# vqdang/hover_net

Measured on AMD Instinct MI355X. Metric: tiles/sec (270x270, batch 32) end-to-end incl. watershed, higher is better.
Workload: dtype fp32

## Files before the change

### hover_net_amd/csrc/hvn_api.hip

```cpp
#include <hip/hip_runtime.h>
#include <stdarg.h>
#include <stdio.h>
#include <string.h>

#include <vector>

#include "hvn_kernels.h"

static thread_local char g_err[512] = "";

int hvn_fail(int code, const char *fmt, ...)
{
    va_list ap;
    va_start(ap, fmt);
    vsnprintf(g_err, sizeof(g_err), fmt, ap);
    va_end(ap);
    return code;
}

int hvn_launch_status(int rc, const char *what)
{
    return rc ? hvn_fail(rc, "%s: %s", what, rc == HVN_E_LAUNCH ? "launch failed" : "the launcher refused these arguments") : HVN_OK;
}

// ... 102 lines not shown

static int nbr_common(const char *what, const hvn_op *op, int batch)
{
    const int N = op->x.h;
    if (!op->w || !op->x2.base) return hvn_fail(HVN_E_ARG, "%s: null pointer", what);
    if (batch != 1) return hvn_fail(HVN_E_ARG, "%s: batch %d, not 1", what, batch);
    if (((uintptr_t)op->w & 7) || ((uintptr_t)op->x2.base & 7)) return hvn_fail(HVN_E_ARG, "%s: misaligned table or workspace (8)", what);
    if (N < 1) return hvn_fail(HVN_E_ARG, "%s: N = %d, fewer than one point", what, N);
    if (op->kh < 1 || op->kw < 1) return hvn_fail(HVN_E_ARG, "%s: a grid of %d x %d cells", what, op->kh, op->kw);
    if (N > HVN_NBR_MAX_N) return hvn_fail(HVN_E_SIZE, "%s: N = %d above 2^26", what, N);
    const long cells = (long)op->kh * op->kw;
    if (op->kh > HVN_NBR_MAX_AXIS || op->kw > HVN_NBR_MAX_AXIS || cells > HVN_NBR_MAX_CELLS)
        return hvn_fail(HVN_E_SIZE, "%s: a grid of %d x %d cells, more than 4096 per axis or 2^22 in all", what, op->kh, op->kw);
    if ((long)op->x2.sn < HVN_NBR_WORKSPACE_BYTES(N, cells))
        return hvn_fail(HVN_E_SIZE, "%s: workspace of %ld bytes, %ld needed", what, (long)op->x2.sn, HVN_NBR_WORKSPACE_BYTES(N, cells));
    return 0;
}

int hvn_internal_run_one(const hvn_op *op, int batch, hipStream_t s)
{
    switch (op->kind) {
    case HVN_OP_CONV0: {
        Conv0Args a;
        set_view(op->x, a.img, a.isn, a.isy, a.isx);
        a.isc = op->x.sc ? op->x.sc : 1;
        a.is_f32 = op->x_dtype;
        a.H = op->x.h; a.W = op->x.w;
        a.w = op->w; a.bias = op->bias;
        set_view(op->y, a.y, a.ysn, a.ysy, a.ysx);
        a.N = batch; a.Ho = op->y.h; a.Wo = op->y.w; a.pad = op->pad_t; a.relu = op->relu; a.out_bf16 = op->act_dtype == 1;
        if (op->kh != 7 || op->kw != 7 || op->x.c != 3 || op->y.c != 64 || !op->w || !op->bias || !op->x.base || !op->y.base)
            return hvn_fail(HVN_E_ARG, "conv0: expects 7x7x3->64 with bias, a non-null image and output");
        if (!aligned16(a.y) || !strides_ok(op->y, 3)) return hvn_fail(HVN_E_ARG, "conv0: output view not 16-byte aligned");
        return hvn_launch_status(hvn_launch_conv0(a, s), "conv0");
    }
    case HVN_OP_CONV: {
        ConvArgs a;
        memset(&a, 0, sizeof(a));
        set_view(op->x, a.x, a.xsn, a.xsy, a.xsx);
        a.H = op->x.h; a.W = op->x.w; a.Cin = op->x.c;
        a.w = op->w; a.bias = op->bias;
        a.pre_s = op->pre_scale; a.pre_b = op->pre_shift;
        a.post_s = op->post_scale; a.post_b = op->post_shift;
        set_view(op->res, a.res, a.rsn, a.rsy, a.rsx);
        set_view(op->y, a.y, a.ysn, a.ysy, a.ysx);
        a.N = batch; a.Ho = op->y.h; a.Wo = op->y.w; a.Cout = op->cout;
        a.KH = op->kh; a.KW = op->kw; a.stride = op->stride; a.pad_t = op->pad_t; a.pad_l = op->pad_l;
        a.relu = op->relu;
        a.groups = op->groups > 1 ? op->groups : 1;
        set_view(op->x2, a.x2, a.x2sn, a.x2sy, a.x2sx);
        a.Cin2 = a.x2 ? op->x2.c : 0;
        a.stride2 = op->_rsv > 0 ? op->_rsv : 1;
        if (a.x2 && (op->kh != 1 || op->kw != 1 || a.stride != 1 || a.Cin2 % 32 || !aligned16(a.x2) || !strides_ok(op->x2, 3) ||
                     a.pre_s || (long)(a.Ho - 1) * a.stride2 >= op->x2.h || (long)(a.Wo - 1) * a.stride2 >= op->x2.w))
            return hvn_fail(HVN_E_ARG, "conv: second input needs a 1x1 stride-1 op without prologue and a view that covers the output grid");
        a.M = (long)batch * a.Ho * a.Wo;
        if (!a.x || !a.w || !a.y) return hvn_fail(HVN_E_ARG, "conv: null pointer");
        if (a.Cin % 32) return hvn_fail(HVN_E_ARG, "conv: input channels must be a multiple of 32 (got %d)", a.Cin);
        if (!aligned16(a.x) || !aligned16(a.w) || !strides_ok(op->x, 3))
            return hvn_fail(HVN_E_ARG, "conv: input view / weights not 16-byte aligned");
        if ((a.pre_s && !aligned16(a.pre_s)) || (a.pre_b && !aligned16(a.pre_b)) || (!a.pre_s != !a.pre_b))
            return hvn_fail(HVN_E_ARG, "conv: prologue vectors must be 16-byte aligned and come in pairs");
        if (!a.post_s != !a.post_b) return hvn_fail(HVN_E_ARG, "conv: epilogue affine must come in pairs");
        if (op->y.c != op->cout) return hvn_fail(HVN_E_ARG, "conv: output view channels != cout");
        a.nbatch = op->nbatch > 1 ? op->nbatch : 1;
        a.xb = op->batch_stride[0]; a.wb = op->batch_stride[1]; a.yb = op->batch_stride[2];
        if (a.nbatch > 1 && ((a.xb | a.wb | a.yb) & 3)) return hvn_fail(HVN_E_ARG, "conv: batch strides must keep 16-byte alignment");
        const bool bf16 = op->act_dtype == 1;
        if (bf16 && (!strides_ok(op->x, 7) || (a.x2 && !strides_ok(op->x2, 7)) || a.nbatch > 1))
            return hvn_fail(HVN_E_ARG, "conv(bf16): input strides must be multiples of 8 elements; no batched launch");
        if (g_prof) prof_mark(s);
        const bool x3 = op->act_dtype == 2 || op->act_dtype == 3;
        if (x3 && (a.groups > 1 || (a.nbatch > 1 && (a.wb & 7)))) return hvn_fail(HVN_E_ARG, "conv(bf16x3): no grouped convs; batch stride of the planes must keep 16-byte alignment");
        int rc;
        if (bf16 && (op->tile_n == 896 || op->tile_n == 640))
            rc = hvn_launch_conv_bf16g(a, op->tile_n == 896 ? 256 : 128, s);
        else if (bf16)
            rc = hvn_launch_conv_bf16(a, op->tile_n, s);
        else if (x3 && (op->tile_n == 896 || op->tile_n == 640))
            rc = hvn_launch_conv_x3g(a, op->tile_n == 896 ? 256 : 128, op->act_dtype == 3 ? 6 : 9, s);
        else
            rc = x3 ? hvn_launch_conv_x3(a, op->tile_n, op->act_dtype == 3 ? 6 : 9, s) : hvn_launch_conv(a, op->tile_n, s);
        if (g_prof) prof_mark(s);
        if (rc) return hvn_fail(rc, "conv: launch failed (tile_n=%d)", op->tile_n);
        return HVN_OK;
    }
    case HVN_OP_CHAIN: {
        ChainArgs a;
        memset(&a, 0, sizeof(a));
        set_view(op->x, a.x, a.xsn, a.xsy, a.xsx);
        a.K1 = op->x.c;
        set_view(op->x2, a.x2, a.x2sn, a.x2sy, a.x2sx);
        a.K1b = a.x2 ? op->x2.c : 0;
        a.stride2 = op->_rsv > 0 ? op->_rsv : 1;
        a.w1 = op->w;
        set_view(op->res, a.res, a.rsn, a.rsy, a.rsx);
        set_view(op->y, a.y, a.ysn, a.ysy, a.ysx);
        a.C = op->cout;
        a.post_s = op->post_scale; a.post_b = op->post_shift;
        a.pre_s = op->pre_scale; a.pre_b = op->pre_shift;
        a.w2 = op->w2; a.bias2 = op->bias2; a.relu2 = 1;
        set_view(op->y2, a.y2, a.y2sn, a.y2sy, a.y2sx);
        a.N2 = op->cout2;
        a.N = batch; a.Ho = op->y.h; a.Wo = op->y.w;
        a.M = (long)batch * a.Ho * a.Wo;
        a.bm = op->tile_n == 64 ? 64 : 128;
        const bool cx3 = op->act_dtype == 2 || op->act_dtype == 3;
        const bool cbf = op->act_dtype == 1;
        if (op->act_dtype != 0 && !cx3 && !cbf) return hvn_fail(HVN_E_ARG, "chain: act_dtype 0 (fp32), 1 (bf16) or 2 | 3 (fp32 with bf16x3 products)");
        const char *form = cbf ? " (bf16)" : "";
        const bool channels_ok = cbf ? hvn_chain_bf16_supported(a.K1, a.K1b, a.C, a.N2) != 0
                                     : hvn_chain_supported(a.C, a.N2) && !(a.K1 % 32 || a.K1b % 32 || a.K1 + a.K1b < 64);
        const long stride_mask = cbf ? 7 : 3;
        if (!a.x || !a.w1 || !a.y || !a.w2 || !a.y2) return hvn_fail(HVN_E_ARG, "chain: null pointer");
        if (op->kh != 1 || op->kw != 1 || op->stride != 1 || op->pad_t || op->pad_l || op->relu || op->bias)
            return hvn_fail(HVN_E_ARG, "chain: the first conv is a plain 1x1 (no bias / relu of its own)");
        if (!channels_ok || op->y.c != a.C || op->y2.c != a.N2)
            return hvn_fail(HVN_E_ARG, "chain%s: needs %s, cout2 in {64, 128} (cout2 = %d)", form,
                            cbf ? "input channels in slabs of 64 (64 or 128 in all), cout % 256 == 0" : "input channels in slabs of 32 (>= 64), cout % 64 == 0", a.N2);
        if (op->x.h != a.Ho || op->x.w != a.Wo || op->y2.h != a.Ho || op->y2.w != a.Wo ||
            (a.x2 && ((long)(a.Ho - 1) * a.stride2 >= op->x2.h || (long)(a.Wo - 1) * a.stride2 >= op->x2.w)))
            return hvn_fail(HVN_E_ARG, "chain: views do not cover the output grid");
        if (a.res && (a.rsn != a.ysn || a.rsy != a.ysy || a.rsx != a.ysx || op->res.c != a.C))
            return hvn_fail(HVN_E_ARG, "chain: the residual view must have the output's strides");
        if (!aligned16(a.x) || !aligned16(a.w1) || !aligned16(a.w2) || !aligned16(a.y) || !aligned16(a.y2) || (a.res && !aligned16(a.res)) ||
            (a.x2 && !aligned16(a.x2)) || !strides_ok(op->x, stride_mask) || !strides_ok(op->y, stride_mask) || !strides_ok(op->y2, stride_mask) ||
            !strides_ok(op->x2, stride_mask))
            return hvn_fail(HVN_E_ARG, "chain%s: views / weights not 16-byte aligned", form);
        if ((!a.pre_s != !a.pre_b) || (!a.post_s != !a.post_b) || (a.pre_s && (!aligned16(a.pre_s) || !aligned16(a.pre_b))) ||
            (a.post_s && (!aligned16(a.post_s) || !aligned16(a.post_b))) || (a.bias2 && !aligned16(a.bias2)))
            return hvn_fail(HVN_E_ARG, "chain: per-channel vectors must be 16-byte aligned and come in pairs");
        if (g_prof) prof_mark(s);
        int rc;
        if (cbf)
            rc = hvn_launch_conv_chain_bf16(a, s);
        else if (cx3 && op->tile_n == 1152)
            rc = hvn_launch_conv_chain_x3r(a, op->act_dtype == 3 ? 6 : 9, s);
        else
            rc = cx3 ? hvn_launch_conv_chain_x3(a, op->act_dtype == 3 ? 6 : 9, s) : hvn_launch_conv_chain(a, s);
        if (g_prof) prof_mark(s);
        if (rc) return hvn_fail(rc, "chain%s: launch failed (cout2=%d)", form, a.N2);
        return HVN_OK;
    }
    case HVN_OP_WINO_IN:
    case HVN_OP_WINO_OUT: {
        WinoArgs a;
        const bool in = op->kind == HVN_OP_WINO_IN;
        set_view(op->x, a.x, a.xsn, a.xsy, a.xsx);
        set_view(op->y, a.y, a.ysn, a.ysy, a.ysx);
        a.mat = op->w; a.bias = op->bias;
        a.N = batch; a.H = in ? op->x.h : op->y.h; a.W = in ? op->x.w : op->y.w; a.C = in ? op->x.c : op->y.c;
        a.ty = op->kh; a.tx = op->kw; a.pad = op->pad_t; a.relu = op->relu;
        a.accum = (!in && op->res.base != nullptr) ? 1 : 0;
        a.lo = nullptr; a.lsn = a.lsy = a.lsx = 0;
        if (in && op->res.base) {
            set_view(op->res, a.lo, a.lsn, a.lsy, a.lsx);
            if (op->res.h * 2 != op->x.h || op->res.w * 2 != op->x.w || op->res.c != op->x.c || !aligned16(a.lo) || !strides_ok(op->res, 3))
                return hvn_fail(HVN_E_ARG, "wino_in: the half-resolution input must be x.h/2 x x.w/2 x x.c and 16-byte aligned");
        }
        if (a.accum && op->res.base != op->y.base) return hvn_fail(HVN_E_ARG, "wino_out: res must alias y (accumulate in place)");
        const int n2 = in ? op->y.h : op->x.h;
        if (op->stride > 1 && op->_rsv > 1) {
            a.m = op->stride; a.r = op->_rsv;
        } else {
            a.m = n2 == 36 ? 2 : n2 == 64 ? 4 : n2 == 100 ? 6 : 0; a.r = 5;
        }
// ... 346 lines not shown
```

### hover_net_amd/csrc/hvn_conv.hip

```cpp
#include <hip/hip_runtime.h>
#include <stdint.h>
#include <stdio.h>
#include <stdlib.h>

#include <vector>

#include <type_traits>

#include "hvn_conv_common.h"

#define BK 32
#define LDS_LD 32
#ifndef HVN_TRACE_FINE
#define HVN_TRACE_FINE 0
#endif
#define HVN_TRACE_WORDS (HVN_TRACE_FINE ? 8 : 4)

template <int BM, int BN, int WAVES_M, int WAVES_N, bool PADDED, bool GROUPED = false, bool HAS_PRE = true, bool HAS_X2 = false>
__global__ __launch_bounds__(256, (BN <= 64 && BM <= 128) ? 3 : 2) void hvn_conv_igemm_f32(ConvArgs p)
{
    unsigned long long t_start = 0, t_kend = 0;
    if (p.dbg) t_start = __builtin_readcyclecounter();
    if (p.nbatch > 1) {
        p.x += (long)blockIdx.y * p.xb;
// ... 359 lines not shown
            ++e_oy;
        }
        while (e_oy >= (unsigned)p.Ho) {
            e_oy -= (unsigned)p.Ho;
            ++e_n;
        }
        const int rr = erow0 + it * RPP;
        f32x4 v = *(const f32x4 *)(ep + rr * EP_LD + ecol);
        v.x = fmaxf(v.x + bias.x, relu_lo);
        v.y = fmaxf(v.y + bias.y, relu_lo);
        v.z = fmaxf(v.z + bias.z, relu_lo);
        v.w = fmaxf(v.w + bias.w, relu_lo);
        v += rall[it];
        v.x = fmaxf(fmaf(v.x, qs.x, qb.x), post_lo);
        v.y = fmaxf(fmaf(v.y, qs.y, qb.y), post_lo);
        v.z = fmaxf(fmaf(v.z, qs.z, qb.z), post_lo);
        v.w = fmaxf(fmaf(v.w, qs.w, qb.w), post_lo);
        vout[it] = v;
    }
#pragma unroll
    for (int it = 0; it < NIT; ++it) asm volatile("" : "+v"(vout[it]), "+v"(yoffs[it]));
    __builtin_amdgcn_sched_barrier(0);
#if HVN_TRACE_FINE
    if (p.dbg) t_f[2] = __builtin_readcyclecounter();
#endif
#pragma unroll
    for (int it = 0; it < NIT; ++it)
        if (oks[it]) *(f32x4 *)(p.y + yoffs[it]) = vout[it];
#if HVN_TRACE_FINE
    if (p.dbg) t_f[3] = __builtin_readcyclecounter();
#endif
    if (p.dbg && tid == 0) {
        asm volatile("s_waitcnt vmcnt(0)" ::: "memory");
        unsigned long long *d = p.dbg + (unsigned long long)HVN_TRACE_WORDS * (blockIdx.x + (unsigned long long)gridDim.x * blockIdx.y);
#if HVN_TRACE_FINE
        d[4] = t_f[0];
        d[5] = t_f[1];
        d[6] = t_f[2];
        d[7] = t_f[3];
#endif
        d[0] = t_start;
        d[1] = t_kend;
        d[2] = __builtin_readcyclecounter();
        d[3] = (unsigned long long)__builtin_amdgcn_s_getreg(4 | (0 << 6) | ((32 - 1) << 11)) |
               ((unsigned long long)__builtin_amdgcn_s_getreg(6 | (0 << 6) | ((8 - 1) << 11)) << 32);
    }
}

template <int BM, int BN, int WAVES_M, int WAVES_N, bool PADDED, bool GROUPED = false, bool HAS_PRE = true, bool HAS_X2 = false>
static int launch_conv(const ConvArgs &a, hipStream_t stream)
{
    ConvArgs p = a;
    static unsigned long long *dbg_buf = nullptr;
    static int dbg_on = -1;
    if (dbg_on < 0) {
        dbg_on = hvn_env_str("HVN_CONV_TRACE") ? 1 : 0;
        if (dbg_on) hipMalloc(&dbg_buf, HVN_TRACE_WORDS * 8 * (size_t)(1 << 20));
    }
    p.dbg = dbg_on ? dbg_buf : nullptr;
    p.m_tiles = (p.M + BM - 1) / BM;
    p.n_tiles = (p.Cout + BN - 1) / BN;
    constexpr size_t stage_fl = (size_t)2 * (BM + BN) * LDS_LD, ep_fl = (size_t)BM * (BN + 4);
    const size_t lds = (stage_fl > ep_fl ? stage_fl : ep_fl) * sizeof(float);
    static std::atomic<unsigned long long> attr_done{0};
    auto kern = hvn_conv_igemm_f32<BM, BN, WAVES_M, WAVES_N, PADDED, GROUPED, HAS_PRE, HAS_X2>;
    if (hvn_max_lds_once((const void *)kern, (int)lds, attr_done)) return HVN_E_LAUNCH;
    const long groups = (p.m_tiles + 7) / 8;
    const long grid = groups * 8 * p.n_tiles;
    if (grid <= 0 || grid > 0x7fffffffL) return HVN_E_ARG;
    hipLaunchKernelGGL(kern, dim3((unsigned)grid, p.nbatch > 1 ? p.nbatch : 1), dim3(256), lds, stream, p);
    if (dbg_on && grid * (p.nbatch > 1 ? p.nbatch : 1) <= (1 << 20)) {
        hipStreamSynchronize(stream);
        const size_t n = (size_t)grid * (p.nbatch > 1 ? p.nbatch : 1);
        std::vector<unsigned long long> h(HVN_TRACE_WORDS * n);
        hipMemcpy(h.data(), dbg_buf, 8 * HVN_TRACE_WORDS * n, hipMemcpyDeviceToHost);
        if (FILE *f = fopen(hvn_env_str("HVN_CONV_TRACE"), "wb")) {
            fwrite(h.data(), 8, h.size(), f);
            fclose(f);
        }
    }
    return hipGetLastError() == hipSuccess ? HVN_OK : HVN_E_LAUNCH;
}

int hvn_launch_dense_grouped(const ConvArgs &a, hipStream_t stream);

int hvn_launch_conv(const ConvArgs &a, int tile_n, hipStream_t stream)
{
    if (a.Cin % BK != 0 || a.Cin <= 0 || a.Cout % 4 != 0) return HVN_E_ARG;
    const int bm = tile_n == 320 ? 256 : 128;
    if (!hvn_conv_reach_ok(a, bm, 4, 256, true, false)) return HVN_E_ARG;
    if ((long)(a.Cout + 128) * a.KH * a.KW * a.Cin * 4 >= (1L << 32)) return HVN_E_ARG;
    const bool padded = hvn_conv_padded(a);
    if (padded && a.pre_s) return HVN_E_ARG;
    if (a.x2) {
        if (padded || a.Cin2 % BK) return HVN_E_ARG;
        if (tile_n == 128) return launch_conv<128, 128, 2, 2, false, false, false, true>(a, stream);
        if (tile_n == 64) return launch_conv<128, 64, 4, 1, false, false, false, true>(a, stream);
        return HVN_E_ARG;
    }
    switch (tile_n) {
    case 128:
        if (!a.pre_s)
            return padded ? launch_conv<128, 128, 2, 2, true, false, false>(a, stream) : launch_conv<128, 128, 2, 2, false, false, false>(a, stream);
        return padded ? launch_conv<128, 128, 2, 2, true>(a, stream) : launch_conv<128, 128, 2, 2, false>(a, stream);
    case 64:
        if (!a.pre_s)
            return padded ? launch_conv<128, 64, 4, 1, true, false, false>(a, stream) : launch_conv<128, 64, 4, 1, false, false, false>(a, stream);
        return padded ? launch_conv<128, 64, 4, 1, true>(a, stream) : launch_conv<128, 64, 4, 1, false>(a, stream);
    case 320:
        if (!a.pre_s)
            return padded ? launch_conv<256, 64, 4, 1, true, false, false>(a, stream) : launch_conv<256, 64, 4, 1, false, false, false>(a, stream);
        return padded ? launch_conv<256, 64, 4, 1, true>(a, stream) : launch_conv<256, 64, 4, 1, false>(a, stream);
    case 32:
        if (a.groups == 4 && a.Cin == 128 && a.Cout == 32 && a.stride == 1 && !padded && !a.pre_s && !a.res && !a.post_s && a.nbatch <= 1 &&
            a.KH == a.KW && (a.KH == 5 || a.KH == 3))
            return hvn_launch_dense_grouped(a, stream);
        if (a.groups == 4 && a.Cin == 128 && a.Cout == 32)
            return padded ? launch_conv<128, 32, 4, 1, true, true>(a, stream) : launch_conv<128, 32, 4, 1, false, true>(a, stream);
        if (a.groups != 1 && !(a.groups == 4 && a.Cin == 128 && a.Cout == 32)) return HVN_E_ARG;
        return padded ? launch_conv<128, 32, 4, 1, true>(a, stream) : launch_conv<128, 32, 4, 1, false>(a, stream);
    default: return HVN_E_ARG;
    }
}

#define DG_TH 8
#define DG_TW 16
#define DG_PP 68
template <int KS>
__global__ __launch_bounds__(256, 2) void hvn_dense_grouped_f32(const ConvArgs p, int tiles_x, int tiles_y)
{
    constexpr int PH = DG_TH + KS - 1, PW = DG_TW + KS - 1;
    extern __shared__ __attribute__((aligned(16))) float dg_patch[];
    const int tid = threadIdx.x, lane = tid & 63, wave = tid >> 6;
    const int l15 = lane & 15, q = lane >> 4;
    int bid = blockIdx.x;
    const int gp = bid & 1;
    bid >>= 1;
    const int tx = bid % tiles_x;
    bid /= tiles_x;
    const int ty = bid % tiles_y;
    const int n = bid / tiles_y;
    const int oy0 = ty * DG_TH, ox0 = tx * DG_TW;
    const float *xin = p.x + (long)n * p.xsn + gp * 64;
    for (int i = tid; i < PH * PW * 16; i += 256) {
        const int c4 = i & 15, pix = i >> 4;
        const int py = pix / PW, px = pix - py * PW;
        const int iy = oy0 + py, ix = ox0 + px;
        f32x4 v = {0.f, 0.f, 0.f, 0.f};
        if (iy < p.H && ix < p.W) v = *(const f32x4 *)(xin + (long)iy * p.xsy + (long)ix * p.xsx + c4 * 4);
        *(f32x4 *)(dg_patch + pix * DG_PP + c4 * 4) = v;
    }
    const int gl = wave & 1, half = wave >> 1;
    const int g = 2 * gp + gl;
    const bool bvalid = l15 < 8;
    const float *wrow = p.w + ((long)(8 * g + (bvalid ? l15 : 0)) * 4 + g) * (KS * KS) * 32 + 8 * q;
    constexpr int TAPS = KS * KS;
    f32x4 wb[4][2];
#pragma unroll
    for (int t = 0; t < 4; ++t) wb[t][0] = wb[t][1] = (f32x4){0.f, 0.f, 0.f, 0.f};
    if (bvalid) {
#pragma unroll
        for (int t = 0; t < 3 && t < TAPS; ++t) {
            wb[t][0] = *(const f32x4 *)(wrow + t * 32);
            wb[t][1] = *(const f32x4 *)(wrow + t * 32 + 4);
        }
    }
    f32x4 acc[4];
#pragma unroll
    for (int m = 0; m < 4; ++m) acc[m] = (f32x4){0.f, 0.f, 0.f, 0.f};
    __syncthreads();
    const float *abase = dg_patch + ((4 * half) * PW + l15) * DG_PP + 32 * gl + 8 * q;
#pragma unroll
    for (int tap = 0; tap < TAPS; ++tap) {
        const int r = tap / KS, s2 = tap % KS;
        if (bvalid && tap + 3 < TAPS) {
            wb[(tap + 3) & 3][0] = *(const f32x4 *)(wrow + (tap + 3) * 32);
            wb[(tap + 3) & 3][1] = *(const f32x4 *)(wrow + (tap + 3) * 32 + 4);
        }
        const float *a = abase + (r * PW + s2) * DG_PP;
        f32x4 a0[4], a1[4];
#pragma unroll
        for (int m = 0; m < 4; ++m) {
            a0[m] = *(const f32x4 *)(a + m * PW * DG_PP);
            a1[m] = *(const f32x4 *)(a + m * PW * DG_PP + 4);
        }
        const f32x4 b0 = wb[tap & 3][0], b1 = wb[tap & 3][1];
#pragma unroll
        for (int e = 0; e < 4; ++e)
#pragma unroll
            for (int m = 0; m < 4; ++m) acc[m] = __builtin_amdgcn_mfma_f32_16x16x4f32(a0[m][e], b0[e], acc[m], 0, 0, 0);
#pragma unroll
        for (int e = 0; e < 4; ++e)
#pragma unroll
            for (int m = 0; m < 4; ++m) acc[m] = __builtin_amdgcn_mfma_f32_16x16x4f32(a1[m][e], b1[e], acc[m], 0, 0, 0);
    }
    if (bvalid) {
        const int co = 8 * g + l15;
        const float bias = p.bias ? p.bias[co] : 0.f;
        const float lo = p.relu ? 0.f : -__builtin_inff();
#pragma unroll
        for (int m = 0; m < 4; ++m) {
            const int oy = oy0 + 4 * half + m;
#pragma unroll
// ... 163 lines not shown
    const float lo = p.relu ? 0.f : -__builtin_inff();
    const float *acol = dg_patch + (2 * l15) * DG_PP + 32 * gl + 8 * q;
    __syncthreads();
    for (int ty = ty0; ty < ty1; ++ty) {
        const int oy0 = ty * DG2_TH;
        f32x4 pf[NPF];
        const bool more = ty + 1 < ty1;
        const int ny0 = oy0 + DG2_TH + PH - 4;
        if (more) {
#pragma unroll
            for (int j = 0; j < NPF; ++j) {
                const int i = tid + 256 * j;
                const int c4 = i & 15, pix = i >> 4;
                const int py = pix / PW, px = pix - py * PW;
                const int iy = ny0 + py, ix = ox0 + px;
                pf[j] = (f32x4){0.f, 0.f, 0.f, 0.f};
                if (i < NEW && iy < p.H && ix < p.W) pf[j] = *(const f32x4 *)(xin + (long)iy * p.xsy + (long)ix * p.xsx + c4 * 4);
            }
        }
        f32x4 wb[4][2];
#pragma unroll
        for (int t = 0; t < 3; ++t) load_w(t, wb[t][0], wb[t][1]);
        f32x4 acc[2] = {{0.f, 0.f, 0.f, 0.f}, {0.f, 0.f, 0.f, 0.f}};
        const int r0 = oy0 + 2 * half;
#pragma unroll
        for (int t2 = 0; t2 < TAPS2; ++t2) {
            const int tr = t2 / (KS + 1), tc = t2 % (KS + 1);
            if (t2 + 3 < TAPS2) load_w(t2 + 3, wb[(t2 + 3) & 3][0], wb[(t2 + 3) & 3][1]);
            f32x4 a0[2], a1[2];
#pragma unroll
            for (int m = 0; m < 2; ++m) {
                const float *a = acol + (((r0 + m + tr) & 7) * PW + tc) * DG_PP;
                a0[m] = *(const f32x4 *)(a);
                a1[m] = *(const f32x4 *)(a + 4);
            }
            const f32x4 b0 = wb[t2 & 3][0], b1 = wb[t2 & 3][1];
#pragma unroll
            for (int e = 0; e < 4; ++e)
#pragma unroll
                for (int m = 0; m < 2; ++m) acc[m] = __builtin_amdgcn_mfma_f32_16x16x4f32(a0[m][e], b0[e], acc[m], 0, 0, 0);
#pragma unroll
            for (int e = 0; e < 4; ++e)
#pragma unroll
                for (int m = 0; m < 2; ++m) acc[m] = __builtin_amdgcn_mfma_f32_16x16x4f32(a1[m][e], b1[e], acc[m], 0, 0, 0);
        }
#pragma unroll
        for (int m = 0; m < 2; ++m) {
            const int oy = oy0 + 2 * half + m;
#pragma unroll
            for (int i = 0; i < 4; ++i) {
                const int ox = ox0 + 2 * (4 * q + i) + dx;
                if (oy < p.Ho && ox < p.Wo) p.y[(long)n * p.ysn + (long)oy * p.ysy + (long)ox * p.ysx + ch] = fmaxf(acc[m][i] + bias, lo);
            }
        }
        if (more) {
            __syncthreads();
#pragma unroll
            for (int j = 0; j < NPF; ++j) {
                const int i = tid + 256 * j;
                const int c4 = i & 15, pix = i >> 4;
                const int py = pix / PW, px = pix - py * PW;
                if (i < NEW) *(f32x4 *)(dg_patch + (((ny0 + py) & 7) * PW + px) * DG_PP + c4 * 4) = pf[j];
            }
            __syncthreads();
        }
    }
}

template <int KS>
static int launch_dense_grouped3(const ConvArgs &a, int run, hipStream_t stream)
{
    const int tiles_x = (a.Wo + DG2_TW - 1) / DG2_TW, tiles_y = (a.Ho + DG2_TH - 1) / DG2_TH;
    const int runs = (tiles_y + run - 1) / run;
    const size_t lds = (size_t)8 * (DG2_TW + KS - 1) * DG_PP * sizeof(float);
    static std::atomic<unsigned long long> attr_done{0};
    auto kern = hvn_dense_grouped3_f32<KS>;
    if (hvn_max_lds_once((const void *)kern, (int)lds, attr_done)) return HVN_E_LAUNCH;
    const long grid = 2L * tiles_x * runs * a.N;
    if (grid <= 0 || grid > 0x7fffffffL) return HVN_E_ARG;
    hipLaunchKernelGGL(kern, dim3((unsigned)grid), dim3(256), lds, stream, a, tiles_x, tiles_y, run, runs);
    return hipGetLastError() == hipSuccess ? HVN_OK : HVN_E_LAUNCH;
}

int hvn_launch_dense_grouped(const ConvArgs &a, hipStream_t stream)
{
    const int wide = ((a.Wo + 31) / 32 * 32) * 100 <= a.Wo * 155;
    const int form = wide ? (a.Ho >= 50 ? 3 : 2) : 1;
    if (form == 3) {
        constexpr int run = 4;
        if (a.KH == 5) return launch_dense_grouped3<5>(a, run, stream);
        if (a.KH == 3) return launch_dense_grouped3<3>(a, run, stream);
        return HVN_E_ARG;
    }
    if (form == 2) {
        if (a.KH == 5) return launch_dense_grouped2<5>(a, stream);
        if (a.KH == 3) return launch_dense_grouped2<3>(a, stream);
        return HVN_E_ARG;
    }
    if (a.KH == 5) return launch_dense_grouped<5>(a, stream);
    if (a.KH == 3) return launch_dense_grouped<3>(a, stream);
    return HVN_E_ARG;
}
```

### hover_net_amd/csrc/hvn_kernels.h

```cpp
#pragma once
#include <hip/hip_runtime.h>
#include <stdint.h>

#include <atomic>

#include "hvn_env.h"
#include "hvn_error.h"

static inline int hvn_max_lds_once(const void *kern, int bytes, std::atomic<unsigned long long> &done)
{
    int dev = 0;
    if (hipGetDevice(&dev) != hipSuccess) return HVN_E_LAUNCH;
    const unsigned long long bit = 1ull << (dev & 63);
    if (done.load(std::memory_order_acquire) & bit) return HVN_OK;
    if (hipFuncSetAttribute(kern, hipFuncAttributeMaxDynamicSharedMemorySize, bytes) != hipSuccess) return HVN_E_LAUNCH;
    done.fetch_or(bit, std::memory_order_release);
    return HVN_OK;
}

struct ConvArgs {
    const float *x;
    long xsn, xsy, xsx;
    int H, W, Cin;
    const float *w;
    const float *bias, *pre_s, *pre_b, *post_s, *post_b;
    const float *res;
    long rsn, rsy, rsx;
    float *y;
    long ysn, ysy, ysx;
    int N, Ho, Wo, Cout, KH, KW, stride, pad_t, pad_l, relu;
    long M;
    long m_tiles;
    int n_tiles;
    int groups;
    const float *x2;
    long x2sn, x2sy, x2sx;
    int Cin2, stride2;
    int nbatch;
    unsigned long long *dbg;
    long xb, wb, yb;
};

int hvn_launch_conv(const ConvArgs &a, int tile_n, hipStream_t stream);

static __device__ __forceinline__ int hvn_m_tile(int xcd, int seq_m, int groups, bool contiguous)
{
    return contiguous ? xcd * groups + seq_m : seq_m * 8 + xcd;
}

struct ChainArgs {
    const float *x;
    long xsn, xsy, xsx;
    int K1;
    const float *x2;
    long x2sn, x2sy, x2sx;
    int K1b, stride2;
    const float *w1;
    const float *res;
    long rsn, rsy, rsx;
    float *y;
    long ysn, ysy, ysx;
    int C;
    const float *post_s, *post_b, *pre_s, *pre_b;
    const float *w2;
    const float *bias2;
    int relu2;
    float *y2;
    long y2sn, y2sy, y2sx;
    int N2;
    int N, Ho, Wo;
    long M;
    int bm;
    unsigned long long *dbg;
};
int hvn_launch_conv_chain(const ChainArgs &a, hipStream_t stream);
int hvn_chain_supported(int c, int n2);
int hvn_chain_bf16_supported(int k1, int k1b, int c, int n2);
int hvn_launch_conv_chain_bf16(const ChainArgs &a, hipStream_t stream);
int hvn_launch_conv_chain_x3(const ChainArgs &a, int terms, hipStream_t stream);
int hvn_chain_x3r_supported(const ChainArgs &a);
int hvn_launch_conv_chain_x3r(const ChainArgs &a, int terms, hipStream_t stream);
int hvn_launch_conv_bf16(const ConvArgs &a, int tile_n, hipStream_t stream);
int hvn_launch_conv_bf16g(const ConvArgs &a, int bm, hipStream_t stream);
int hvn_launch_conv_x3(const ConvArgs &a, int tile_n, int terms, hipStream_t stream);
int hvn_launch_conv_x3g(const ConvArgs &a, int bm, int terms, hipStream_t stream);
int hvn_conv_x3g_supported(const ConvArgs &a, int bm);
int hvn_launch_split_x3(const float *src, uint16_t *dst, long granules, hipStream_t stream);

struct Conv0Args {
    const void *img;
    long isn, isy, isx, isc;
    int is_f32;
    int H, W;
    const float *w;
    const float *bias;
    float *y;
    long ysn, ysy, ysx;
    int N, Ho, Wo, pad;
    int relu;
    int out_bf16;
};
int hvn_launch_conv0(const Conv0Args &a, hipStream_t stream);

struct UpAddArgs {
    const float *lo;
    long lsn, lsy, lsx;
    const float *skip;
    long ssn, ssy, ssx;
    float *y;
    long ysn, ysy, ysx;
    int N, H, W, C;
    int bf16;
};
int hvn_launch_upadd(const UpAddArgs &a, hipStream_t stream);

struct HeadArgs {
    const float *x;
    long xsn, xsy, xsx;
    const float *w;
    const float *bias;
    float *y;
    int N, H, W, Cout;
    int in_bf16;
};
int hvn_launch_head(const HeadArgs &a, hipStream_t stream);

// ... 311 lines not shown
```

### hover_net_amd/lib.py

```python
import ctypes
import os
import re
import subprocess

from .knobs import knob

_HERE = os.path.dirname(os.path.abspath(__file__))
LIB_PATH = os.path.join(_HERE, "libhvn_hip.so")
VARIANTS = {
    "fullepi": ("-DHVN_X3G_FULL_EPI=1",),
    "prev": (),
    "trace": ("-DHVN_TRACE_FINE=1",),
}
CSRC = os.path.join(_HERE, "csrc")
HEADERS = ("hvn_conv_common.h", "hvn_env.h", "hvn_error.h", "hvn_kernels.h")
SOURCES = ("hvn_conv.hip", "hvn_conv_chain.hip", "hvn_conv_chain_x3.hip", "hvn_conv_chain_x3r.hip", "hvn_conv_bf16.hip", "hvn_conv_bf16g.hip", "hvn_conv_chain_bf16.hip", "hvn_conv_x3.hip", "hvn_conv_x3g.hip", "hvn_net_ops.hip", "hvn_postproc.hip", "hvn_api.hip", "hvn_train.hip", "hvn_wgrad_x3.hip", "hvn_targets.hip", "hvn_wsi_merge.hip",
           "hvn_augment.hip", "hvn_train_api.hip", "hvn_contour.cpp", "hvn_contour_dev.hip", "hvn_metrics.hip", "hvn_valid.hip", "hvn_overlay.hip", "hvn_resample.hip", "hvn_tissue.hip", "hvn_viz.hip", "hvn_features.hip", "hvn_tta.hip", "hvn_stain.hip", "hvn_neighbours.hip", "hvn_clusters.hip", "hvn_density.hip", "hvn_pairs.hip", "hvn_regions.hip")
HIPCC_FLAGS = ("--offload-arch=gfx950", "-O3", "-std=c++17", "-fPIC", "-shared", "-ffp-contract=off",
               "-fvisibility=hidden", "-Wno-unused-value", "-pthread")


class HvnError(RuntimeError):
    pass


HEADER = os.path.join(os.path.dirname(_HERE), "include", "hvn.h")
_SCALARS = {"int": ctypes.c_int, "int32_t": ctypes.c_int32, "int64_t": ctypes.c_int64, "size_t": ctypes.c_size_t, "long": ctypes.c_long,
            "float": ctypes.c_float, "double": ctypes.c_double}


def parse_header(text):
    text = re.sub(r"/\*.*?\*/|//[^\n]*|^[ \t]*#[^\n]*", " ", text, flags=re.S | re.M)
    structs, protos = {}, {}
    for chunk in re.split(r"\btypedef\s+struct\b", text)[1:]:
        m = re.match(r"\s*(\w+)\s*\{([^{}]*)\}\s*(\w+)\s*;", chunk)
        if not m or m.group(1) != m.group(3):
            raise HvnError("hvn.h: cannot read `typedef struct %s ...`" % " ".join(chunk.split())[:60])
        name, body, fields = m.group(1), m.group(2), []
        for decl in filter(None, (d.strip() for d in body.split(";"))):
            base, _, rest = re.sub(r"\bconst\b", " ", decl).strip().partition(" ")
            for d in rest.split(","):
                m = re.fullmatch(r"\s*(\*?)\s*(\w+)\s*(?:\[(\d+)\])?\s*", d)
                if m and m.group(1):
                    t = ctypes.POINTER(structs[base]) if base in structs else ctypes.c_void_p
                else:
                    t = structs.get(base) or _SCALARS.get(base)
                if not m or t is None:
                    raise HvnError("hvn.h: cannot map `%s` of struct %s" % (decl, name))
                fields.append((m.group(2), t * int(m.group(3)) if m.group(3) else t))
        structs[name] = type(name, (ctypes.Structure,), {"_fields_": fields})
    for decl in re.findall(r"\bHVN_API\b([^;]*);", text):
        m = re.fullmatch(r"([^()]*?)(\w+)\s*\(([^()]*)\)\s*", decl)
        if not m:
            raise HvnError("hvn.h: cannot read `HVN_API %s`" % " ".join(decl.split()))
        ret, name, args = " ".join(m.group(1).split()), m.group(2), m.group(3)
        restype = ctypes.c_char_p if ret == "const char *" else _SCALARS.get(ret)
        params = [ctypes.c_void_p if "*" in a or "[" in a else _SCALARS.get(" ".join(a.replace("const ", " ").split()[:-1]))
                  for a in ([] if args.strip() == "void" else args.split(","))]
        if restype is None or None in params:
            raise HvnError("hvn.h: cannot map `%s %s(%s)`" % (ret, name, " ".join(args.split())))
        protos[name] = (restype, params)
    return structs, protos


STRUCTS, PROTOS = parse_header(open(HEADER).read())
globals().update(STRUCTS)
EXPORTS = tuple(PROTOS)


def source_id():
    import hashlib

    h = hashlib.sha256()
    for f in sorted(SOURCES) + list(HEADERS):
        h.update(f.encode())
        h.update(open(os.path.join(CSRC, f), "rb").read())
    h.update(open(os.path.join(os.path.dirname(_HERE), "include", "hvn.h"), "rb").read())
    h.update(" ".join(HIPCC_FLAGS).encode())
    return h.hexdigest()[:16]


def _built_id(path):
    if not os.path.exists(path):
        return None
    data = open(path, "rb").read()
    i = data.find(b"hvn-build-id:")
    if i < 0:
        return None
    j = data.find(b"\0", i)
    return data[i + 13:j].decode(errors="replace")


_HIPCC_VERSION = None


def _hipcc_version():
    global _HIPCC_VERSION
    if _HIPCC_VERSION is None:
        try:
# ... 125 lines not shown
```

### hover_net_amd/tune.py

```python
import math

import torch

from . import lib as L
from .knobs import KNOBS, knob
from .plan import OP_CHAIN, OP_CONV, _tile_n

MARGIN = 0.985
X3G_256, X3G_128 = 128 + 0x300, 128 + 0x200
X3R = 128 + 0x400
T256X64 = 64 + 0x100
OPTIONAL = (X3G_256, X3G_128, X3R)
WGRAD_TARGETS = (1536, 1024, 768, 512, 384)
WG_SLOTS = 512

CACHE = {}


def tile_select():
    v = knob("HVN_TILE_SELECT")
    if v not in ("auto", "model", "0"):
        raise ValueError("HVN_TILE_SELECT=%r: auto, model or 0" % v)
    return v


def time_launch(launch, reps=3, runs=1):
    reps = max(1, int(knob("HVN_TUNE_REPS") or reps))
    e0, e1 = torch.cuda.Event(enable_timing=True), torch.cuda.Event(enable_timing=True)
    best = float("inf")
    for r in range(reps + 1):
        e0.record()
        for _ in range(runs):
            launch()
        e1.record()
        e1.synchronize()
        if r:
            best = min(best, e0.elapsed_time(e1) / runs)
    return best


def choose(cache, key, candidates, measure, margin=MARGIN, optional=OPTIONAL):
    key = tuple(key) + (tuple(candidates),)
    if key not in cache:
        t = {}
        for c in candidates:
            try:
                t[c] = measure(c)
            except L.HvnError:
                if c not in optional:
                    raise
                t[c] = float("inf")
        base = candidates[0]
        best = min(candidates[1:], key=t.get)
        cache[key] = (best if t[best] < margin * t[base] else base, t[base], t[best], t)
    return cache[key]


def forced_form(o):
    if o.kind == OP_CHAIN:
        return X3R if knob("HVN_CHAIN_X3R") == "force" else None
    v = knob("HVN_BF16G_FORCE" if o.act_dtype == 1 else "HVN_X3G_FORCE")
    return int(v) if v else None


def pick(cache, key, candidates, measure, forced=None, optional=OPTIONAL, **kw):
    if forced in optional and forced in candidates[1:]:
        try:
            measure(forced)
            return forced
        except L.HvnError:
            return candidates[0]
    return choose(cache, key, candidates, measure, optional=optional, **kw)[0]


def entries(family, device=None):
    return [(k, v) for k, v in CACHE.items() if k[1] == family and (device is None or k[0] == str(device))]


def launch_key(device, family, o, batch):
    return (str(device), family, int(batch), o.kh, o.kw, o.stride, o.pad_t, o.x.c, o.cout, o.cout2, o.y.h, o.y.w, o.x.h, o.x.w, bool(o.res.base),
            bool(o.pre_scale), bool(o.post_scale), int(o.nbatch), int(o.x2.c) if o.x2.base else 0, int(o.act_dtype), int(o.groups))


def x3g_forms_for(o):
    want = knob("HVN_X3G")
    if want == "0" or o.cout < 128 or o.groups > 1:
        return ()
    forms = []
    for code, bm, na in ((X3G_256, 256, 3), (X3G_128, 128, 2)):
        if want not in ("1", str(code)):
            continue
        if o.pre_scale and bm == 256 and na * bm * 128 + 2 * 3 * 128 * 64 + 2 * o.x.c * 4 > 160 * 1024:
            continue
        forms.append(code)
    return tuple(forms)


def candidates(o):
    x3, bf16 = o.act_dtype in (2, 3), o.act_dtype == 1
    if o.kind == OP_CHAIN:
        if x3:
            if knob("HVN_CHAIN_X3R") == "0" or o.x.c != 64 or (o.x2.base and (o.x2.c != 64 or o.res.base or o.cout2 != 64)):
                return ()
            return (128, X3R)
        return () if bf16 else (128, 64)
    if o.kind != OP_CONV or o.groups > 1:
        return ()
    static = _tile_n(o.cout)
    if bf16:
        if static != 128 or o.pre_scale or o.nbatch > 1 or knob("HVN_BF16G") == "0":
            return ()
        return (128, X3G_256, X3G_128)
    if static == 128:
        return (128, 64) + (x3g_forms_for(o) if x3 else ())
    if static == 64 and not x3 and not o.x2.base:
        return (64, T256X64)
    return ()


def pick_tile_n(op, batch):
    if op.tile_n != 128 or tile_select() == "0":
        return op.tile_n
    force = knob("HVN_FORCE_TILE_N")
    if force:
        return int(force)
    slots64 = int(knob("HVN_WG_SLOTS_64"))
    cost64 = float(knob("HVN_NARROW_COST"))
    m_tiles = math.ceil(batch * op.y.h * op.y.w / 128.0)
    nb = int(op.extra.get("nbatch", 1))
    wide = math.ceil(m_tiles * math.ceil(op.cout / 128.0) * nb / WG_SLOTS)
    narrow = math.ceil(m_tiles * math.ceil(op.cout / 64.0) * nb / slots64) * cost64
    return 64 if narrow < wide else 128
```

Baseline: 756.0.

## Add double-buffered DMA persistent kernel for grouped dense-unit convs, autotuned

Adds a new persistent kernel for the 4-group 128->32 dense-unit convolutions. Each 512-thread workgroup keeps the group's weights resident in LDS and uses buffer-to-LDS DMA to prefetch the next input tile while MFMA runs on the current one. It also exposes the existing dense_grouped forms by tile_n code, and the autotuner measures the DMA form against the default, keeping it only when it wins. The goal is to hide global-load latency and cut per-tile weight reloads, at the cost of one workgroup per CU and a persistent grid.

Measured after the change: 769.1, median of 6. +1.7%, better.

```diff
diff --git a/hover_net_amd/csrc/hvn_api.hip b/hover_net_amd/csrc/hvn_api.hip
--- a/hover_net_amd/csrc/hvn_api.hip
+++ b/hover_net_amd/csrc/hvn_api.hip
@@ -208,6 +208,10 @@
         else
             rc = x3 ? hvn_launch_conv_x3(a, op->tile_n, op->act_dtype == 3 ? 6 : 9, s) : hvn_launch_conv(a, op->tile_n, s);
         if (g_prof) prof_mark(s);
+        if (rc == HVN_E_ARG && !bf16 && !x3 && op->tile_n >= HVN_DENSE_FORM(1) && op->tile_n <= HVN_DENSE_FORM(4) && (op->tile_n & 0xff) == 32)
+            return hvn_fail(rc, "conv: dense-unit form %d (tile_n=%d) does not exist for this launch: 128 -> 32 channels in 4 groups, 5x5 | 3x3, stride 1, "
+                                "no padding, prologue, residual or post vectors, one problem%s", (op->tile_n - 32) >> 8, op->tile_n,
+                            op->tile_n == HVN_DENSE_FORM(4) ? "; 16-byte aligned input view within 2^31 bytes per sample" : "");
         if (rc) return hvn_fail(rc, "conv: launch failed (tile_n=%d)", op->tile_n);
         return HVN_OK;
     }
diff --git a/hover_net_amd/csrc/hvn_conv.hip b/hover_net_amd/csrc/hvn_conv.hip
--- a/hover_net_amd/csrc/hvn_conv.hip
+++ b/hover_net_amd/csrc/hvn_conv.hip
@@ -465,7 +465,12 @@
     return hipGetLastError() == hipSuccess ? HVN_OK : HVN_E_LAUNCH;
 }
 
-int hvn_launch_dense_grouped(const ConvArgs &a, hipStream_t stream);
+int hvn_launch_dense_grouped(const ConvArgs &a, int form, hipStream_t stream);
+static bool dense_unit_launch(const ConvArgs &a, bool padded)
+{
+    return a.groups == 4 && a.Cin == 128 && a.Cout == 32 && a.stride == 1 && !padded && !a.pre_s && !a.res && !a.post_s && a.nbatch <= 1 &&
+           a.KH == a.KW && (a.KH == 5 || a.KH == 3);
+}
 
 int hvn_launch_conv(const ConvArgs &a, int tile_n, hipStream_t stream)
 {
@@ -495,13 +500,17 @@
             return padded ? launch_conv<256, 64, 4, 1, true, false, false>(a, stream) : launch_conv<256, 64, 4, 1, false, false, false>(a, stream);
         return padded ? launch_conv<256, 64, 4, 1, true>(a, stream) : launch_conv<256, 64, 4, 1, false>(a, stream);
     case 32:
-        if (a.groups == 4 && a.Cin == 128 && a.Cout == 32 && a.stride == 1 && !padded && !a.pre_s && !a.res && !a.post_s && a.nbatch <= 1 &&
-            a.KH == a.KW && (a.KH == 5 || a.KH == 3))
-            return hvn_launch_dense_grouped(a, stream);
+        if (dense_unit_launch(a, padded)) return hvn_launch_dense_grouped(a, 0, stream);
         if (a.groups == 4 && a.Cin == 128 && a.Cout == 32)
             return padded ? launch_conv<128, 32, 4, 1, true, true>(a, stream) : launch_conv<128, 32, 4, 1, false, true>(a, stream);
         if (a.groups != 1 && !(a.groups == 4 && a.Cin == 128 && a.Cout == 32)) return HVN_E_ARG;
         return padded ? launch_conv<128, 32, 4, 1, true>(a, stream) : launch_conv<128, 32, 4, 1, false>(a, stream);
+    case HVN_DENSE_FORM(1):
+    case HVN_DENSE_FORM(2):
+    case HVN_DENSE_FORM(3):
+        if (!dense_unit_launch(a, padded)) return HVN_E_ARG;
+        return hvn_launch_dense_grouped(a, (tile_n - 32) >> 8, stream);
+    case HVN_DENSE_FORM(4): return hvn_launch_dense_dma(a, stream);
     default: return HVN_E_ARG;
     }
 }
@@ -831,10 +840,10 @@
     return hipGetLastError() == hipSuccess ? HVN_OK : HVN_E_LAUNCH;
 }
 
-int hvn_launch_dense_grouped(const ConvArgs &a, hipStream_t stream)
+int hvn_launch_dense_grouped(const ConvArgs &a, int forced, hipStream_t stream)
 {
     const int wide = ((a.Wo + 31) / 32 * 32) * 100 <= a.Wo * 155;
-    const int form = wide ? (a.Ho >= 50 ? 3 : 2) : 1;
+    const int form = forced ? forced : wide ? (a.Ho >= 50 ? 3 : 2) : 1;
     if (form == 3) {
         constexpr int run = 4;
         if (a.KH == 5) return launch_dense_grouped3<5>(a, run, stream);
diff --git a/hover_net_amd/csrc/hvn_dense_dma.hip b/hover_net_amd/csrc/hvn_dense_dma.hip
--- /dev/null
+++ b/hover_net_amd/csrc/hvn_dense_dma.hip
@@ -0,0 +1,191 @@
+#include "hvn_conv_common.h"
+
+#define DD_TH 8
+#define DD_TW 16
+
+template <int KS>
+struct DenseDma {
+    static constexpr int PH = DD_TH + KS - 1, PW = DD_TW + KS - 1;
+    static constexpr int PWP = PW | 1;
+    static constexpr int SLOTS = PH * PWP * 8;
+    static constexpr int NDW = (SLOTS + 255) / 256;
+    static constexpr int BUF = NDW * 4 * 1024;
+    static constexpr int TAPS2 = KS * (KS + 1);
+    static constexpr int WPITCH = 36 * 4;
+    static constexpr int WTAP = 8 * WPITCH;
+    static constexpr int P_OFF = (KS * KS * WTAP + 1023) / 1024 * 1024;
+    static constexpr int LDS = P_OFF + 4 * BUF;
+    static_assert(LDS <= 160 * 1024, "one workgroup per CU");
+};
+
+template <int KS>
+__global__ __launch_bounds__(512, 1) void hvn_dense_dma_f32(const ConvArgs p, int tiles_x, int tiles_y, int tiles, int units)
+{
+    using D = DenseDma<KS>;
+    constexpr int PWP = D::PWP, NDW = D::NDW, TAPS2 = D::TAPS2;
+    extern __shared__ __attribute__((aligned(1024))) unsigned char dd_lds[];
+    const int tid = threadIdx.x, lane = tid & 63;
+    const int wave8 = __builtin_amdgcn_readfirstlane(tid >> 6);
+    const int half = wave8 >> 2, wave = wave8 & 3;
+    const int l15 = lane & 15, q = lane >> 4;
+    const int g = blockIdx.x & 3;
+
+    for (int i = tid; i < KS * KS * 8 * 8; i += 512) {
+        const int piece = i & 7, wc = (i >> 3) & 7, tap = i >> 6;
+        const f32x4 v = *(const f32x4 *)(p.w + ((long)(8 * g + wc) * 4 + g) * (KS * KS) * 32 + tap * 32 + piece * 4);
+        *(f32x4 *)(dd_lds + tap * D::WTAP + wc * D::WPITCH + piece * 16) = v;
+    }
+
+    unsigned x_voff[NDW];
+    int x_py[NDW], x_px[NDW];
+#pragma unroll
+    for (int jj = 0; jj < NDW; ++jj) {
+        const int slot = (wave * NDW + jj) * 64 + lane;
+        const int pix = slot >> 3;
+        const int py = pix / PWP, px = pix - py * PWP;
+        const int piece = (slot & 7) ^ ((px >> 1) & 7);
+        const bool in_patch = slot < D::SLOTS && px < D::PW;
+        x_py[jj] = in_patch ? py : (1 << 20);
+        x_px[jj] = px;
+        x_voff[jj] = (unsigned)(((long)py * p.xsy + (long)px * p.xsx + g * 32 + piece * 4) * 4);
+    }
+    unsigned char *const my_patch = dd_lds + D::P_OFF + half * 2 * D::BUF;
+    auto tile_of = [&](int u, int &n, int &oy0, int &ox0) {
+        int r = 2 * (u >> 2) + half;
+        const bool live = r < tiles;
+        r = live ? r : 0;
+        const int tx = r % tiles_x;
+        r /= tiles_x;
+        const int ty = r % tiles_y;
+        n = __builtin_amdgcn_readfirstlane(r / tiles_y);
+        oy0 = __builtin_amdgcn_readfirstlane(ty * DD_TH);
+        ox0 = __builtin_amdgcn_readfirstlane(tx * DD_TW);
+        return live;
+    };
+    auto issue = [&](int u, int buf) {
+        int n, oy0, ox0;
+        const bool live = tile_of(u, n, oy0, ox0);
+        const __amdgpu_buffer_rsrc_t rsrc_x = hvn_buf(p.x + (long)n * p.xsn);
+        const int soff = __builtin_amdgcn_readfirstlane((int)(((long)oy0 * p.xsy + (long)ox0 * p.xsx) * 4));
+        const int hrem = live ? p.H - oy0 : 0, wrem = p.W - ox0;
+#pragma unroll
+        for (int jj = 0; jj < NDW; ++jj) {
+            const bool ok = x_py[jj] < hrem && x_px[jj] < wrem;
+            hvn_dma16(rsrc_x, (lds_ptr_t)(my_patch + buf * D::BUF + (wave * NDW + jj) * 1024), ok ? x_voff[jj] : HVN_OOB, soff);
+        }
+    };
+
+    const int co = l15 & 7, dx = l15 >> 3;
+    const int w_lane0 = co * D::WPITCH + q * 32, w_lane1 = w_lane0 - dx * D::WTAP;
+    constexpr int NK = KS / 2 + 1;
+    unsigned a_lane[NK][2];
+#pragma unroll
+    for (int k = 0; k < NK; ++k)
+#pragma unroll
+        for (int h = 0; h < 2; ++h)
+            a_lane[k][h] = (unsigned)(((2 * wave + (l15 >> 3)) * PWP + 2 * (l15 & 7)) * 128 + (((2 * q + h) ^ (((l15 & 7) + k) & 7)) << 4));
+    const int ch = 8 * g + co;
+    const float bias = p.bias ? p.bias[ch] : 0.f;
+    const float lo = p.relu ? 0.f : -__builtin_inff();
+    const int e_oy = 2 * wave + (q >> 1), e_ox = 2 * (4 * (q & 1)) + dx;
+
+    const int G = (int)gridDim.x;
+    int u = (int)blockIdx.x;
+    if (u >= units) return;
+    issue(u, 0);
+    asm volatile("s_waitcnt vmcnt(0) lgkmcnt(0)" ::: "memory");
+    __builtin_amdgcn_s_barrier();
+    for (int buf = 0; u < units; u += G, buf ^= 1) {
+        if (u + G < units) issue(u + G, buf ^ 1);
+        const unsigned char *patch = my_patch + buf * D::BUF;
+        auto read_ab = [&](int t2, f32x4(&f)[4]) {
+            const int tr = t2 / (KS + 1), tc = t2 % (KS + 1);
+            f[0] = *(const f32x4 *)(patch + a_lane[tc >> 1][0] + (tr * PWP + tc) * 128);
+            f[1] = *(const f32x4 *)(patch + a_lane[tc >> 1][1] + (tr * PWP + tc) * 128);
+            const int ftap = tr * KS + (tc == KS ? KS - 1 : tc);
+            const int wl = ((tc == 0 || tc == KS) ? w_lane0 : w_lane1) + ftap * D::WTAP;
+            f[2] = *(const f32x4 *)(dd_lds + wl);
+            f[3] = *(const f32x4 *)(dd_lds + wl + 16);
+        };
+        f32x4 acc = {0.f, 0.f, 0.f, 0.f};
+        f32x4 fr[2][4];
+        read_ab(0, fr[0]);
+#pragma unroll
+        for (int t2 = 0; t2 < TAPS2; ++t2) {
+            const int tc = t2 % (KS + 1);
+            if (t2 + 1 < TAPS2) read_ab(t2 + 1, fr[(t2 + 1) & 1]);
+            __builtin_amdgcn_sched_barrier(0);
+            const f32x4 a0 = fr[t2 & 1][0], a1 = fr[t2 & 1][1];
+            f32x4 b0 = fr[t2 & 1][2], b1 = fr[t2 & 1][3];
+            if (tc == 0 || tc == KS) {
+                const bool zero = tc == 0 ? dx != 0 : dx == 0;
+#pragma unroll
+                for (int e = 0; e < 4; ++e) {
+                    b0[e] = zero ? 0.f : b0[e];
+                    b1[e] = zero ? 0.f : b1[e];
+                }
+            }
+#pragma unroll
+            for (int e = 0; e < 4; ++e) acc = __builtin_amdgcn_mfma_f32_16x16x4f32(a0[e], b0[e], acc, 0, 0, 0);
+#pragma unroll
+            for (int e = 0; e < 4; ++e) acc = __builtin_amdgcn_mfma_f32_16x16x4f32(a1[e], b1[e], acc, 0, 0, 0);
+            __builtin_amdgcn_sched_barrier(0);
+        }
+        asm volatile("s_waitcnt vmcnt(0) lgkmcnt(0)" ::: "memory");
+        {
+            int n, oy0, ox0;
+            const bool live = tile_of(u, n, oy0, ox0);
+            const int oy = oy0 + e_oy;
+            float *yrow = p.y + (long)n * p.ysn + (long)oy * p.ysy + ch;
+#pragma unroll
+            for (int i = 0; i < 4; ++i) {
+                const int ox = ox0 + e_ox + 2 * i;
+                if (live && oy < p.Ho && ox < p.Wo) yrow[(long)ox * p.ysx] = fmaxf(acc[i] + bias, lo);
+            }
+        }
+        __builtin_amdgcn_s_barrier();
+    }
+}
+
+int hvn_dense_dma_supported(const ConvArgs &a)
+{
+    if (!(a.groups == 4 && a.Cin == 128 && a.Cout == 32 && a.stride == 1 && !hvn_conv_padded(a) && !a.pre_s && !a.res && !a.post_s && a.nbatch <= 1 &&
+          a.KH == a.KW && (a.KH == 5 || a.KH == 3)))
+        return 0;
+    if (((uintptr_t)a.x & 15) || (a.xsn & 3) || (a.xsy & 3) || (a.xsx & 3) || ((uintptr_t)a.w & 15)) return 0;
+    if (a.xsy < 0 || a.xsx < 0) return 0;
+    const long span = ((long)(a.H + DD_TH + a.KH) * a.xsy + (long)(a.W + DD_TW + a.KW) * a.xsx + 128) * 4;
+    if (span >= (1L << 31)) return 0;
+    const long tiles = (long)a.N * ((a.Ho + DD_TH - 1) / DD_TH) * ((a.Wo + DD_TW - 1) / DD_TW);
+    return tiles > 0 && tiles < (1L << 28);
+}
+
+template <int KS>
+static int launch_dense_dma(const ConvArgs &a, hipStream_t stream)
+{
+    const int tiles_x = (a.Wo + DD_TW - 1) / DD_TW, tiles_y = (a.Ho + DD_TH - 1) / DD_TH;
+    const long tiles = (long)a.N * tiles_y * tiles_x;
+    const long units = 4 * ((tiles + 1) / 2);
+    constexpr size_t lds = DenseDma<KS>::LDS;
+    static std::atomic<unsigned long long> attr_done{0};
+    static std::atomic<int> slots{0};
+    auto kern = hvn_dense_dma_f32<KS>;
+    if (hvn_max_lds_once((const void *)kern, (int)lds, attr_done)) return HVN_E_LAUNCH;
+    int res = slots.load(std::memory_order_relaxed);
+    if (!res) {
+        int dev = 0, cus = 0;
+        if (hipGetDevice(&dev) != hipSuccess || hipDeviceGetAttribute(&cus, hipDeviceAttributeMultiprocessorCount, dev) != hipSuccess || cus < 4)
+            return HVN_E_LAUNCH;
+        res = cus & ~3;
+        slots.store(res, std::memory_order_relaxed);
+    }
+    const long grid = units < res ? units : (long)res;
+    hipLaunchKernelGGL(kern, dim3((unsigned)grid), dim3(512), lds, stream, a, tiles_x, tiles_y, (int)tiles, (int)units);
+    return hipGetLastError() == hipSuccess ? HVN_OK : HVN_E_LAUNCH;
+}
+
+int hvn_launch_dense_dma(const ConvArgs &a, hipStream_t stream)
+{
+    if (!hvn_dense_dma_supported(a)) return HVN_E_ARG;
+    return a.KH == 5 ? launch_dense_dma<5>(a, stream) : launch_dense_dma<3>(a, stream);
+}
diff --git a/hover_net_amd/csrc/hvn_kernels.h b/hover_net_amd/csrc/hvn_kernels.h
--- a/hover_net_amd/csrc/hvn_kernels.h
+++ b/hover_net_amd/csrc/hvn_kernels.h
@@ -42,6 +42,9 @@
 };
 
 int hvn_launch_conv(const ConvArgs &a, int tile_n, hipStream_t stream);
+#define HVN_DENSE_FORM(f) (32 + 0x100 * (f))
+int hvn_dense_dma_supported(const ConvArgs &a);
+int hvn_launch_dense_dma(const ConvArgs &a, hipStream_t stream);
 
 static __device__ __forceinline__ int hvn_m_tile(int xcd, int seq_m, int groups, bool contiguous)
 {
diff --git a/hover_net_amd/lib.py b/hover_net_amd/lib.py
--- a/hover_net_amd/lib.py
+++ b/hover_net_amd/lib.py
@@ -14,7 +14,7 @@
 }
 CSRC = os.path.join(_HERE, "csrc")
 HEADERS = ("hvn_conv_common.h", "hvn_env.h", "hvn_error.h", "hvn_kernels.h")
-SOURCES = ("hvn_conv.hip", "hvn_conv_chain.hip", "hvn_conv_chain_x3.hip", "hvn_conv_chain_x3r.hip", "hvn_conv_bf16.hip", "hvn_conv_bf16g.hip", "hvn_conv_chain_bf16.hip", "hvn_conv_x3.hip", "hvn_conv_x3g.hip", "hvn_net_ops.hip", "hvn_postproc.hip", "hvn_api.hip", "hvn_train.hip", "hvn_wgrad_x3.hip", "hvn_targets.hip", "hvn_wsi_merge.hip",
+SOURCES = ("hvn_conv.hip", "hvn_dense_dma.hip", "hvn_conv_chain.hip", "hvn_conv_chain_x3.hip", "hvn_conv_chain_x3r.hip", "hvn_conv_bf16.hip", "hvn_conv_bf16g.hip", "hvn_conv_chain_bf16.hip", "hvn_conv_x3.hip", "hvn_conv_x3g.hip", "hvn_net_ops.hip", "hvn_postproc.hip", "hvn_api.hip", "hvn_train.hip", "hvn_wgrad_x3.hip", "hvn_targets.hip", "hvn_wsi_merge.hip",
            "hvn_augment.hip", "hvn_train_api.hip", "hvn_contour.cpp", "hvn_contour_dev.hip", "hvn_metrics.hip", "hvn_valid.hip", "hvn_overlay.hip", "hvn_resample.hip", "hvn_tissue.hip", "hvn_viz.hip", "hvn_features.hip", "hvn_tta.hip", "hvn_stain.hip", "hvn_neighbours.hip", "hvn_clusters.hip", "hvn_density.hip", "hvn_pairs.hip", "hvn_regions.hip")
 HIPCC_FLAGS = ("--offload-arch=gfx950", "-O3", "-std=c++17", "-fPIC", "-shared", "-ffp-contract=off",
                "-fvisibility=hidden", "-Wno-unused-value", "-pthread")
diff --git a/hover_net_amd/tune.py b/hover_net_amd/tune.py
--- a/hover_net_amd/tune.py
+++ b/hover_net_amd/tune.py
@@ -10,7 +10,8 @@
 X3G_256, X3G_128 = 128 + 0x300, 128 + 0x200
 X3R = 128 + 0x400
 T256X64 = 64 + 0x100
-OPTIONAL = (X3G_256, X3G_128, X3R)
+DENSE_F1, DENSE_F2, DENSE_F3, DENSE_DMA = 32 + 0x100, 32 + 0x200, 32 + 0x300, 32 + 0x400
+OPTIONAL = (X3G_256, X3G_128, X3R, DENSE_DMA)
 WGRAD_TARGETS = (1536, 1024, 768, 512, 384)
 WG_SLOTS = 512
 
@@ -104,6 +105,10 @@
                 return ()
             return (128, X3R)
         return () if bf16 else (128, 64)
+    if o.kind == OP_CONV and o.groups == 4:
+        dense = (not x3 and not bf16 and o.x.c == 128 and o.cout == 32 and o.kh == o.kw and o.kh in (5, 3) and o.stride == 1
+                 and o.pad_t == 0 and o.pad_l == 0 and o.tile_n in (32, DENSE_DMA))
+        return (32, DENSE_DMA) if dense else ()
     if o.kind != OP_CONV or o.groups > 1:
         return ()
     static = _tile_n(o.cout)
```
